# slinderman/pyglm

Measured on AMD Instinct MI355X. Metric: Gibbs sweeps/sec (full resample_model), higher is better.
Workload: dtype f64 (likelihood Gram: exact integer arithmetic on 13 i8 residue planes, CRT back to f64)

## Files before the change

pyglm_amd/csrc/pgl_gemm.hip:

```cpp
#include "pgl_common.h"
#include <type_traits>

namespace {

constexpr int BK = 16;
constexpr int PAD = 16;

template <int WM, int WN, int WZ, bool WEIGHTED, int STAGES = 2>
struct Cfg {
    static constexpr int BM = WM * 64, BN = WN * 64;
    static constexpr int SA = BM + PAD, SB = BN + PAD;
    static constexpr int THREADS = WM * WN * WZ * 64;
    static constexpr int A_ELEMS = BK * SA, B_ELEMS = BK * SB, W_ELEMS = WEIGHTED ? BK * WZ : 0;
    static constexpr int STAGE = A_ELEMS + B_ELEMS + W_ELEMS;
    static constexpr size_t LDS_BYTES = (size_t)STAGES * STAGE * sizeof(double);
    static constexpr int A_LD = (BK * BM / 2) / THREADS, B_LD = (BK * BN / 2) / THREADS;
    static_assert((BK * BM / 2) % THREADS == 0 && (BK * BN / 2) % THREADS == 0, "tile/threads mismatch");
};

__device__ __forceinline__ int isqrt_tri(int t) {
    int r = (int)((__builtin_sqrt(8.0 * (double)t + 1.0) - 1.0) * 0.5);
    while ((long)(r + 1) * (r + 2) / 2 <= t) ++r;
    while ((long)r * (r + 1) / 2 > t) --r;
    return r;
}

__device__ __forceinline__ void block_sync_lds() {
    asm volatile("s_waitcnt lgkmcnt(0)" ::: "memory");
    __builtin_amdgcn_s_barrier();
    asm volatile("" ::: "memory");
}

template <int WM, int WN, int WZ, bool WEIGHTED, int STAGES, bool DMA = false, bool CINIT = false, bool SQ = false>
__device__ __forceinline__ void gemm_item(const PglGemmArgs& g, const long w, double* smem) {
    using C = Cfg<WM, WN, WZ, WEIGHTED, STAGES>;
    const int ntm = (g.M + C::BM - 1) / C::BM;
    int tile, batch, tm, tn;
    if (g.nbatch > 1) {
        if (WEIGHTED || (g.strideA == 0 && g.strideB == 0)) {
            tile = (int)(w / g.nbatch); batch = (int)(w % g.nbatch);
        } else {
            const int ntn_ = (g.N + C::BN - 1) / C::BN;
            const long ntiles = g.tri ? (long)ntm * (ntm + 1) / 2 : (long)ntm * ntn_;
            batch = (int)(w / ntiles); tile = (int)(w % ntiles);
        }
    } else { tile = (int)w; batch = 0; }
    if (g.tri) { tm = isqrt_tri(tile); tn = tile - tm * (tm + 1) / 2; if (g.tri == 2) { const int s_ = tm; tm = tn; tn = s_; } }
    else { tm = tile % ntm; tn = tile / ntm; }
    int Mv = g.M, Nv = g.N;
    if (g.batch_dim) {
        const int d = g.batch_dim[batch] - g.dim_off;
        if (g.dim_mode == 0) { Mv = d; Nv = d; }
        else if (g.dim_mode == 1) Nv = d;
        else if (g.dim_mode == 2) Mv = d;
        else { Mv = g.M < d ? g.M : d; Nv = d; }
    }
    if (tm * C::BM >= Mv || tn * C::BN >= Nv) return;

    int K = g.K;
    if (g.batch_k) { K = g.batch_k[batch]; if (K <= 0) return; }
    const int nkt = K / BK;

    const int tid = threadIdx.x, lane = tid & 63, wave = tid >> 6;
    const int wz = wave / (WM * WN), wmn = wave % (WM * WN), wm = wmn / WN, wn = wmn % WN;
    const int m0 = tm * C::BM, n0 = tn * C::BN;

    const double* __restrict__ Ab = g.A + (long)batch * g.strideA;
    const long roff_ = g.batch_row_off ? (long)g.batch_row_off[batch] : 0;
    const double* __restrict__ Bb = g.B + (long)batch * g.strideB + roff_ * g.ldb;
    const int zg = batch * WZ + wz;
    const bool zvalid = !WEIGHTED || zg < g.nz_total;

    d2_t ra[C::A_LD], rb[C::B_LD];
    double rw = 0.0;
    const unsigned long long aflip = (CINIT && g.alpha < 0.0) ? 0x8000000000000000ull : 0ull;
    typedef unsigned long long u2_t __attribute__((ext_vector_type(2)));
    auto signed_a = [&](d2_t v) { return __builtin_bit_cast(d2_t, __builtin_bit_cast(u2_t, v) ^ u2_t{aflip, aflip}); };
    unsigned oa_[C::A_LD], ob_[C::B_LD], ow_ = 0;
    const char* ka_ = reinterpret_cast<const char*>(Ab);
    const char* kb_ = reinterpret_cast<const char*>(Bb);
    const char* kw_ = reinterpret_cast<const char*>(g.W);
#pragma unroll
    for (int i = 0; i < C::A_LD; ++i) {
        const int p = tid + i * C::THREADS, r = p / (C::BM / 2), c = (p % (C::BM / 2)) * 2;
        int col = m0 + c;
        col = col < g.a_cols ? col : g.a_cols - 2;
        oa_[i] = (unsigned)(((long)r * g.lda + col) * 8);
    }
#pragma unroll
    for (int i = 0; i < C::B_LD; ++i) {
        const int p = tid + i * C::THREADS, r = p / (C::BN / 2), c = (p % (C::BN / 2)) * 2;
        int col = n0 + c;
        col = col < g.b_cols ? col : g.b_cols - 2;
        ob_[i] = (unsigned)(((long)r * g.ldb + col) * 8);
    }
    if (WEIGHTED) {
        const int t_ = tid < BK * WZ ? tid : 0, r = t_ / WZ, z = t_ % WZ;
        int zc = batch * WZ + z;
        zc = zc < g.nz_total ? zc : g.nz_total - 1;
        ow_ = (unsigned)(((long)r * g.ldw + zc) * 8);
    }
    const long stepA = (long)BK * g.lda * 8, stepB = (long)BK * g.ldb * 8, stepW = (long)BK * g.ldw * 8;
    auto gload = [&](int) {
#pragma unroll
        for (int i = 0; i < C::A_LD; ++i) ra[i] = *reinterpret_cast<const d2_t*>(ka_ + oa_[i]);
#pragma unroll
        for (int i = 0; i < C::B_LD; ++i) rb[i] = *reinterpret_cast<const d2_t*>(kb_ + ob_[i]);
        if (WEIGHTED && tid < BK * WZ) rw = *reinterpret_cast<const double*>(kw_ + ow_);
        ka_ += stepA; kb_ += stepB; kw_ += stepW;
    };
    auto lstore = [&](int buf) {
        double* As = smem + buf * C::STAGE;
        double* Bs = As + C::A_ELEMS;
#pragma unroll
        for (int i = 0; i < C::A_LD; ++i) {
            const int p = tid + i * C::THREADS, r = p / (C::BM / 2), c = (p % (C::BM / 2)) * 2;
            if constexpr (CINIT) *reinterpret_cast<d2_t*>(As + r * C::SA + c) = signed_a(SQ ? ra[i] * ra[i] : ra[i]);
            else *reinterpret_cast<d2_t*>(As + r * C::SA + c) = SQ ? ra[i] * ra[i] : ra[i];
        }
#pragma unroll
        for (int i = 0; i < C::B_LD; ++i) {
            const int p = tid + i * C::THREADS, r = p / (C::BN / 2), c = (p % (C::BN / 2)) * 2;
            *reinterpret_cast<d2_t*>(Bs + r * C::SB + c) = SQ ? rb[i] * rb[i] : rb[i];
        }
        if (WEIGHTED && tid < BK * WZ) (Bs + C::B_ELEMS)[tid] = rw;
    };

    d4_t acc[4][4];
    const int frow = lane >> 4, fcol = lane & 15;
    const bool interior = CINIT && m0 + C::BM <= Mv && n0 + C::BN <= Nv;
    if constexpr (CINIT) {
        const double* __restrict__ cp = g.C + (long)batch * g.strideC + roff_ * g.ldc + (long)(m0 + wm * 64 + frow) * g.ldc + (n0 + wn * 64 + fcol);
        if (interior) {
#pragma unroll
            for (int i = 0; i < 4; ++i)
#pragma unroll
                for (int r = 0; r < 4; ++r)
#pragma unroll
                    for (int j = 0; j < 4; ++j) acc[i][j][r] = cp[(long)(i * 16 + 4 * r) * g.ldc + j * 16];
        } else {
#pragma unroll
            for (int i = 0; i < 4; ++i)
#pragma unroll
                for (int r = 0; r < 4; ++r)
#pragma unroll
                    for (int j = 0; j < 4; ++j) {
                        const int row = m0 + wm * 64 + i * 16 + frow + 4 * r, col = n0 + wn * 64 + j * 16 + fcol;
                        acc[i][j][r] = (row < Mv && col < Nv) ? cp[(long)(i * 16 + 4 * r) * g.ldc + j * 16] : 0.0;
                    }
        }
    } else {
#pragma unroll
        for (int i = 0; i < 4; ++i)
#pragma unroll
            for (int j = 0; j < 4; ++j) acc[i][j] = d4_t{0.0, 0.0, 0.0, 0.0};
    }
    auto compute = [&](int buf, int kk) {
        const double* As = smem + buf * C::STAGE + wm * 64 + fcol;
        const double* Bs = smem + buf * C::STAGE + C::A_ELEMS + wn * 64 + fcol;
        const double* Ws = smem + buf * C::STAGE + C::A_ELEMS + C::B_ELEMS;
        const int kr = kk * 4 + frow;
        double a[4], b[4];
#pragma unroll
        for (int i = 0; i < 4; ++i) a[i] = As[kr * C::SA + i * 16];
#pragma unroll
        for (int j = 0; j < 4; ++j) b[j] = Bs[kr * C::SB + j * 16];
        if (WEIGHTED) {
            const double wv = Ws[kr * WZ + wz];
#pragma unroll
            for (int i = 0; i < 4; ++i) a[i] *= wv;
        }
#pragma unroll
        for (int i = 0; i < 4; ++i)
#pragma unroll
            for (int j = 0; j < 4; ++j) acc[i][j] = __builtin_amdgcn_mfma_f64_16x16x4f64(a[i], b[j], acc[i][j], 0, 0, 0);
    };

    if constexpr (STAGES == 2) {
        gload(0);
        lstore(0);
        __syncthreads();
        if constexpr (!WEIGHTED) {
            constexpr int NLD = C::A_LD + C::B_LD;
            static_assert(NLD <= 16, "one staged load per MFMA slot of a k-step");
            auto gload_piece = [&](int q) {
                if (q < C::A_LD) ra[q] = *reinterpret_cast<const d2_t*>(ka_ + oa_[q]);
                else rb[q - C::A_LD] = *reinterpret_cast<const d2_t*>(kb_ + ob_[q - C::A_LD]);
            };
            auto lstore_piece = [&](int buf, int q) {
                double* As = smem + buf * C::STAGE;
                double* Bs = As + C::A_ELEMS;
                if (q < C::A_LD) {
                    const int p = tid + q * C::THREADS, r = p / (C::BM / 2), c = (p % (C::BM / 2)) * 2;
                    if constexpr (CINIT) *reinterpret_cast<d2_t*>(As + r * C::SA + c) = signed_a(SQ ? ra[q] * ra[q] : ra[q]);
                    else *reinterpret_cast<d2_t*>(As + r * C::SA + c) = SQ ? ra[q] * ra[q] : ra[q];
                } else {
                    const int i = q - C::A_LD;
                    const int p = tid + i * C::THREADS, r = p / (C::BN / 2), c = (p % (C::BN / 2)) * 2;
                    *reinterpret_cast<d2_t*>(Bs + r * C::SB + c) = SQ ? rb[i] * rb[i] : rb[i];
                }
            };
            auto kstep = [&](int buf, int kk, auto hook) {
                const double* As = smem + buf * C::STAGE + wm * 64 + fcol;
                const double* Bs = smem + buf * C::STAGE + C::A_ELEMS + wn * 64 + fcol;
                const int kr = kk * 4 + frow;
                double a[4], b[4];
#pragma unroll
                for (int i = 0; i < 4; ++i) a[i] = As[kr * C::SA + i * 16];
#pragma unroll
                for (int j = 0; j < 4; ++j) b[j] = Bs[kr * C::SB + j * 16];
#pragma unroll
                for (int m = 0; m < 16; ++m) {
                    acc[m >> 2][m & 3] = __builtin_amdgcn_mfma_f64_16x16x4f64(a[m >> 2], b[m & 3], acc[m >> 2][m & 3], 0, 0, 0);
                    hook(m);
                    __builtin_amdgcn_sched_barrier(0);
                }
            };
            if constexpr (CINIT && NLD <= 8) {
                double fa0[4], fb0[4], fa1[4], fb1[4];
                auto rd_first = [&](int buf) {
                    const double* As = smem + buf * C::STAGE + wm * 64 + fcol;
                    const double* Bs = smem + buf * C::STAGE + C::A_ELEMS + wn * 64 + fcol;
#pragma unroll
                    for (int i = 0; i < 4; ++i) fa0[i] = As[frow * C::SA + i * 16];
#pragma unroll
                    for (int j = 0; j < 4; ++j) fb0[j] = Bs[frow * C::SB + j * 16];
                };
                auto kstep_a = [&](int buf, auto kk_c, auto hook) {
                    constexpr int KK = decltype(kk_c)::value;
                    double (&ca)[4] = (KK & 1) ? fa1 : fa0;
                    double (&cb)[4] = (KK & 1) ? fb1 : fb0;
                    double (&na)[4] = (KK & 1) ? fa0 : fa1;
                    double (&nb)[4] = (KK & 1) ? fb0 : fb1;
                    const double* As = smem + buf * C::STAGE + wm * 64 + fcol;
                    const double* Bs = smem + buf * C::STAGE + C::A_ELEMS + wn * 64 + fcol;
                    const int krn = (KK + 1) * 4 + frow;
#pragma unroll
                    for (int m = 0; m < 16; ++m) {
                        asm volatile("v_mfma_f64_16x16x4_f64 %0, %1, %2, %0" : "+a"(acc[m >> 2][m & 3]) : "v"(ca[m >> 2]), "v"(cb[m & 3]));
                        if constexpr (KK < 3) {
                            if (m < 4) na[m] = As[krn * C::SA + m * 16];
                            else if (m < 8) nb[m - 4] = Bs[krn * C::SB + (m - 4) * 16];
                        }
                        hook(m);
                        __builtin_amdgcn_sched_barrier(0);
                    }
                };
                using K0 = std::integral_constant<int, 0>; using K1 = std::integral_constant<int, 1>;
                using K2 = std::integral_constant<int, 2>; using K3 = std::integral_constant<int, 3>;
                auto nohook = [](int) {};
                rd_first(0);
                asm volatile("s_nop 7\n\ts_nop 7" ::: "memory");
                for (int kt = 0; kt + 1 < nkt; ++kt) {
                    const int buf = kt & 1;
                    kstep_a(buf, K0{}, [&](int m) { if (m >= 8 && m - 8 < NLD) gload_piece(m - 8); });
                    ka_ += stepA; kb_ += stepB;
                    kstep_a(buf, K1{}, nohook);
                    kstep_a(buf, K2{}, nohook);
                    kstep_a(buf, K3{}, [&](int m) { if (m >= 16 - NLD) lstore_piece(buf ^ 1, m - (16 - NLD)); });
                    __syncthreads();
                    rd_first(buf ^ 1);
                }
                {
                    const int buf = (nkt - 1) & 1;
                    kstep_a(buf, K0{}, nohook);
                    kstep_a(buf, K1{}, nohook);
                    kstep_a(buf, K2{}, nohook);
                    kstep_a(buf, K3{}, nohook);
                }
                asm volatile("s_nop 7\n\ts_nop 7\n\ts_nop 7" ::: "memory");
            } else {
            for (int kt = 0; kt + 1 < nkt; ++kt) {
                const int buf = kt & 1;
                kstep(buf, 0, [&](int m) { if (m < NLD) gload_piece(m); });
                ka_ += stepA; kb_ += stepB;
                compute(buf, 1);
                compute(buf, 2);
                kstep(buf, 3, [&](int m) { if (m >= 16 - NLD) lstore_piece(buf ^ 1, m - (16 - NLD)); });
                __syncthreads();
            }
            {
                const int buf = (nkt - 1) & 1;
#pragma unroll
                for (int kk = 0; kk < BK / 4; ++kk) compute(buf, kk);
            }
            }
        } else {
            for (int kt = 0; kt < nkt; ++kt) {
                const int buf = kt & 1;
                if (kt + 1 < nkt) gload(kt + 1);
#pragma unroll
                for (int kk = 0; kk < BK / 4; ++kk) compute(buf, kk);
                if (kt + 1 < nkt) lstore(buf ^ 1);
                __syncthreads();
            }
        }
    } else {
        static_assert(DMA && WEIGHTED && (STAGES == 3 || STAGES == 4), "the 3/4-stage pipeline is the DMA-staged weighted Gram");
        typedef __attribute__((address_space(3))) void* lds_ptr_t;
        typedef const __attribute__((address_space(1))) void* glb_ptr_t;
        static_assert(C::BM == 128 && C::BN == 128 && C::THREADS == 512, "DMA staging is written for the Gram tile");
        const int wv = __builtin_amdgcn_readfirstlane(wave);
        const char* gp[5];
        long gstep[5];
        int loff[5];
        {
            int ca = m0 + lane * 2, cb = n0 + lane * 2;
            ca = ca < g.a_cols ? ca : g.a_cols - 2;
            cb = cb < g.b_cols ? cb : g.b_cols - 2;
#pragma unroll
            for (int p = 0; p < 4; ++p) {
                const int r = wv + 8 * (p >> 1);
                if ((p & 1) == 0) { gp[p] = reinterpret_cast<const char*>(Ab + (long)r * g.lda + ca); gstep[p] = (long)BK * g.lda * 8; loff[p] = r * C::SA * 8; }
                else { gp[p] = reinterpret_cast<const char*>(Bb + (long)r * g.ldb + cb); gstep[p] = (long)BK * g.ldb * 8; loff[p] = (C::A_ELEMS + r * C::SB) * 8; }
            }
            const int dw = wv * 8 + (lane & 7), dbl = dw >> 1, r = dbl / WZ, zq = dbl % WZ;
            int zc = batch * WZ + zq;
            zc = zc < g.nz_total ? zc : g.nz_total - 1;
            gp[4] = reinterpret_cast<const char*>(g.W + (long)r * g.ldw + zc) + 4 * (dw & 1);
            gstep[4] = (long)BK * g.ldw * 8;
            loff[4] = (C::A_ELEMS + C::B_ELEMS) * 8 + wv * 32;
        }
        long gadv[5];
        auto advance = [&](bool adv) {
#pragma unroll
            for (int p = 0; p < 5; ++p) gadv[p] = adv ? gstep[p] : 0;
        };
        auto dma_piece = [&](int stage, int p) {
            char* dst = reinterpret_cast<char*>(smem) + (size_t)stage * C::STAGE * 8 + loff[p];
            if (p < 4) __builtin_amdgcn_global_load_lds((glb_ptr_t)gp[p], (lds_ptr_t)dst, 16, 0, 0);
            else if (lane < 8) __builtin_amdgcn_global_load_lds((glb_ptr_t)gp[4], (lds_ptr_t)dst, 4, 0, 0);
            asm volatile("v_lshl_add_u64 %0, %1, 0, %2" : "=v"(gp[p]) : "v"(gp[p]), "s"(gadv[p]));
        };
        auto dma = [&](int stage) {
#pragma unroll
            for (int p = 0; p < 5; ++p) dma_piece(stage, p);
        };
        advance(1 < nkt);
        dma(0);
        advance(2 < nkt);
        dma(1);
        if constexpr (STAGES == 4) { advance(3 < nkt); dma(2); }
        advance(STAGES < nkt);
        if constexpr (STAGES == 4) asm volatile("s_waitcnt vmcnt(10)" ::: "memory");
        else asm volatile("s_waitcnt vmcnt(5)" ::: "memory");
        __syncthreads();
        int cur = 0;
        {
            const int wq = wmn;
            double pa[2][2][2], pb[2][2][8], pw[2][2];
            auto rdA = [&](int buf, int kk, int i) { return smem[buf * C::STAGE + wq * 32 + fcol + (kk * 4 + frow) * C::SA + i * 16]; };
            auto rdB = [&](int buf, int kk, int j) { return smem[buf * C::STAGE + C::A_ELEMS + fcol + (kk * 4 + frow) * C::SB + j * 16]; };
            auto rdW = [&](int buf, int kk) { return smem[buf * C::STAGE + C::A_ELEMS + C::B_ELEMS + (kk * 4 + frow) * WZ + wz]; };
#pragma unroll
            for (int i = 0; i < 2; ++i) { pa[0][0][i] = rdA(0, 0, i); pa[0][1][i] = rdA(0, 1, i); }
#pragma unroll
            for (int j = 0; j < 8; ++j) pb[0][0][j] = rdB(0, 0, j);
            pw[0][0] = rdW(0, 0); pw[0][1] = rdW(0, 1);
#pragma unroll
            for (int i = 0; i < 2; ++i) { pa[0][0][i] *= pw[0][0]; pa[0][1][i] *= pw[0][1]; }
            for (int kt = 0; kt < nkt; ++kt) {
                const int nxt = (cur == STAGES - 1) ? 0 : cur + 1;
                const int dstage = (cur == 0) ? STAGES - 1 : cur - 1;
                if (kt + STAGES >= nkt) advance(false);
#pragma unroll
                for (int p = 0; p < 2; ++p) {
                    const int ps = p, ns = p ^ 1;
                    const int nbuf = (p == 0) ? cur : nxt, nk = (p == 0) ? 2 : 0;
#pragma unroll
                    for (int m = 0; m < 16; ++m) {
                        const int i = m >> 3, j = m & 7;
                        acc[m >> 2][m & 3] = __builtin_amdgcn_mfma_f64_16x16x4f64(pa[ps][0][i], pb[ps][0][j], acc[m >> 2][m & 3], 0, 0, 0);
                        if (m < 8) pb[ps][1][m] = rdB(cur, 2 * p + 1, m);
                        else if (m < 10) pa[ns][0][m - 8] = rdA(nbuf, nk, m - 8);
                        else if (m == 10) pw[ns][0] = rdW(nbuf, nk);
                        else if (m == 11) pw[ns][1] = rdW(nbuf, nk + 1);
                        else { if (p == 1) dma_piece(dstage, m - 12); }
                        __builtin_amdgcn_sched_barrier(0);
                    }
#pragma unroll
                    for (int m = 0; m < 16; ++m) {
                        const int i = m >> 3, j = m & 7;
                        acc[m >> 2][m & 3] = __builtin_amdgcn_mfma_f64_16x16x4f64(pa[ps][1][i], pb[ps][1][j], acc[m >> 2][m & 3], 0, 0, 0);
                        if (m < 2) pa[ns][1][m] = rdA(nbuf, nk + 1, m);
                        else if (m < 10) pb[ns][0][m - 2] = rdB(nbuf, nk, m - 2);
                        else if (m == 10) { if (p == 1) dma_piece(dstage, 4); }
                        else if (m == 13) {
#pragma unroll
                            for (int q = 0; q < 2; ++q) { pa[ns][0][q] *= pw[ns][0]; pa[ns][1][q] *= pw[ns][1]; }
                        }
                        __builtin_amdgcn_sched_barrier(0);
                    }
                    if (p == 0) {
                        if constexpr (STAGES == 4) asm volatile("s_waitcnt vmcnt(5)" ::: "memory");
                        else asm volatile("s_waitcnt vmcnt(0)" ::: "memory");
                        block_sync_lds();
                    }
                }
                cur = nxt;
            }
        }
    }

    if (!zvalid) return;
    double* __restrict__ Cb = g.C + (WEIGHTED ? (long)zg : (long)batch) * g.strideC + roff_ * g.ldc;
    const double alpha = g.alpha, beta = g.beta;
    constexpr bool WIDE = STAGES >= 3;
    auto roff = [&](int i, int j) { return WIDE ? wmn * 32 + ((4 * i + j) >> 3) * 16 : wm * 64 + i * 16; };
    auto coff = [&](int i, int j) { return WIDE ? ((4 * i + j) & 7) * 16 : wn * 64 + j * 16; };
    if constexpr (CINIT) {
        double* __restrict__ cq = Cb + (long)(m0 + wm * 64 + frow) * g.ldc + (n0 + wn * 64 + fcol);
        if (interior) {
#pragma unroll
            for (int i = 0; i < 4; ++i)
#pragma unroll
                for (int r = 0; r < 4; ++r)
#pragma unroll
                    for (int j = 0; j < 4; ++j) cq[(long)(i * 16 + 4 * r) * g.ldc + j * 16] = acc[i][j][r];
        } else {
#pragma unroll
            for (int i = 0; i < 4; ++i)
#pragma unroll
                for (int r = 0; r < 4; ++r)
#pragma unroll
                    for (int j = 0; j < 4; ++j) {
                        const int row = m0 + wm * 64 + i * 16 + frow + 4 * r, col = n0 + wn * 64 + j * 16 + fcol;
                        if (row < Mv && col < Nv) cq[(long)(i * 16 + 4 * r) * g.ldc + j * 16] = acc[i][j][r];
                    }
        }
        return;
    }
#pragma unroll
    for (int i = 0; i < 4; ++i) {
        double cv[4][4];
        if (beta != 0.0) {
#pragma unroll
            for (int r = 0; r < 4; ++r) {
#pragma unroll
                for (int j = 0; j < 4; ++j) {
                    const int row = m0 + roff(i, j) + frow + 4 * r, col = n0 + coff(i, j) + fcol;
                    cv[r][j] = (row < Mv && col < Nv) ? Cb[(long)row * g.ldc + col] : 0.0;
                }
            }
        }
#pragma unroll
        for (int r = 0; r < 4; ++r) {
#pragma unroll
            for (int j = 0; j < 4; ++j) {
                const int row = m0 + roff(i, j) + frow + 4 * r, col = n0 + coff(i, j) + fcol;
                if (row >= Mv || col >= Nv) continue;
                double v = alpha * acc[i][j][r];
                if (beta != 0.0) v += beta * cv[r][j];
                Cb[(long)row * g.ldc + col] = v;
            }
        }
    }
}

template <int WM, int WN, int WZ, bool WEIGHTED, int STAGES, bool CINIT = false, bool SQ = false>
__global__ __launch_bounds__(WM* WN* WZ * 64, 2) void gemm_tn_f64(PglGemmArgs g) {
    using C = Cfg<WM, WN, WZ, WEIGHTED, STAGES>;
    extern __shared__ __attribute__((aligned(16))) double smem[];
    const int ntm = (g.M + C::BM - 1) / C::BM, ntn = (g.N + C::BN - 1) / C::BN;
    const long total = (long)(g.tri ? ntm * (ntm + 1) / 2 : ntm * ntn) * g.nbatch;
    const long chunk = (total + 7) / 8;
    long w = (long)(blockIdx.x & 7) * chunk + (blockIdx.x >> 3);
    if ((long)(blockIdx.x >> 3) >= chunk || w >= total) return;
    gemm_item<WM, WN, WZ, WEIGHTED, STAGES, false, CINIT, SQ>(g, w, smem);
}

template <int WM, int WN, int WZ, bool WEIGHTED, int STAGES, bool DMA>
__global__ __launch_bounds__(WM* WN* WZ * 64, 2) void gemm_tn_f64_persistent(PglGemmArgs g) {
    using C = Cfg<WM, WN, WZ, WEIGHTED, STAGES>;
    extern __shared__ __attribute__((aligned(16))) double smem[];
    long* ticket = reinterpret_cast<long*>(smem + (size_t)STAGES * C::STAGE);
    const int ntm = (g.M + C::BM - 1) / C::BM, ntn = (g.N + C::BN - 1) / C::BN;
    const long total = (long)(g.tri ? ntm * (ntm + 1) / 2 : ntm * ntn) * g.nbatch;
    const long chunk = (total + 7) / 8;
    unsigned xcc;
    asm volatile("s_getreg_b32 %0, hwreg(HW_REG_XCC_ID)" : "=s"(xcc));
    xcc &= 7u;
    for (;;) {
        __syncthreads();
        if (threadIdx.x == 0) {
            long w = -1;
            for (int hop = 0; hop < 8 && w < 0; ++hop) {
                const int y = (int)((xcc + hop) & 7u);
                const long lo = (long)y * chunk, hi = (lo + chunk < total) ? lo + chunk : total;
                if (lo >= hi) continue;
                const long it = atomicAdd(&g.sched[y], 1);
                if (lo + it < hi) w = lo + it;
            }
            ticket[0] = w;
        }
        __syncthreads();
        const long w = ticket[0];
        if (w < 0) break;
        gemm_item<WM, WN, WZ, WEIGHTED, STAGES, DMA>(g, w, smem);
    }
}

constexpr int FK = 8, FST = 4, FSA = 128 + PAD;
constexpr int F_A = FK * FSA, F_B = FK * FSA, F_W = FK;
constexpr int F_STAGE = F_A + F_B + F_W;
constexpr size_t F_LDS = (size_t)FST * F_STAGE * sizeof(double) + 16;

__device__ __forceinline__ void gram_fine_item(const PglGemmArgs& g, const long w, double* smem) {
    typedef __attribute__((address_space(3))) void* lds_ptr_t;
    typedef const __attribute__((address_space(1))) void* glb_ptr_t;
    const int nz = g.nz_total;
    const int z = (int)(w % nz);
    const int S = g.ksplit > 1 ? g.ksplit : 1;
    const int sl = (int)((w / nz) % S), tile = (int)(w / nz / S);
    const int tm = isqrt_tri(tile), tn = tile - tm * (tm + 1) / 2;
    const int m0 = tm * 128, n0 = tn * 128;
    const long krow0 = S > 1 ? (long)sl * g.ks_rows : 0;
    const int Ks = S > 1 ? (int)((long)g.K - krow0 < g.ks_rows ? (long)g.K - krow0 : g.ks_rows) : g.K;
    const int nkt = Ks / FK;
    const int tid = threadIdx.x, lane = tid & 63, wq = tid >> 6;
    const int frow = lane >> 4, fcol = lane & 15;
    const double* __restrict__ Ab = g.A + krow0 * g.lda;
    const double* __restrict__ Bb = g.B + krow0 * g.ldb;

    const int wv = __builtin_amdgcn_readfirstlane(wq);
    const char* gp[5];
    long gstep[5], gadv[5];
    int loff[5];
    {
        int ca = m0 + lane * 2, cb = n0 + lane * 2;
        ca = ca < g.a_cols ? ca : g.a_cols - 2;
        cb = cb < g.b_cols ? cb : g.b_cols - 2;
#pragma unroll
        for (int p = 0; p < 4; ++p) {
            const int r = wv + 4 * (p >> 1);
            if ((p & 1) == 0) { gp[p] = reinterpret_cast<const char*>(Ab + (long)r * g.lda + ca); gstep[p] = (long)FK * g.lda * 8; loff[p] = r * FSA * 8; }
            else { gp[p] = reinterpret_cast<const char*>(Bb + (long)r * g.ldb + cb); gstep[p] = (long)FK * g.ldb * 8; loff[p] = (F_A + r * FSA) * 8; }
        }
        const int dw = wv * 4 + (lane & 3), r = dw >> 1;
        gp[4] = reinterpret_cast<const char*>(g.W + (krow0 + r) * g.ldw + z) + 4 * (dw & 1);
        gstep[4] = (long)FK * g.ldw * 8;
        loff[4] = (F_A + F_B) * 8 + wv * 16;
    }
    auto advance = [&](bool adv) {
#pragma unroll
        for (int p = 0; p < 5; ++p) gadv[p] = adv ? gstep[p] : 0;
    };
    auto dma_piece = [&](int stage, int p) {
        char* dst = reinterpret_cast<char*>(smem) + (size_t)stage * F_STAGE * 8 + loff[p];
        if (p < 4) __builtin_amdgcn_global_load_lds((glb_ptr_t)gp[p], (lds_ptr_t)dst, 16, 0, 0);
        else if (lane < 4) __builtin_amdgcn_global_load_lds((glb_ptr_t)gp[4], (lds_ptr_t)dst, 4, 0, 0);
        gp[p] += gadv[p];
    };
    auto dma = [&](int stage) {
#pragma unroll
        for (int p = 0; p < 5; ++p) dma_piece(stage, p);
    };

    d4_t acc[4][4];
#pragma unroll
    for (int i = 0; i < 4; ++i)
#pragma unroll
        for (int j = 0; j < 4; ++j) acc[i][j] = d4_t{0.0, 0.0, 0.0, 0.0};

    advance(1 < nkt); dma(0);
    advance(2 < nkt); dma(1);
    advance(3 < nkt); dma(2);
    asm volatile("s_waitcnt vmcnt(5)" ::: "memory");
    block_sync_lds();

    double pa[2][2][2], pb[2][2][8], pw[2][2];
    auto rdA = [&](int buf, int kk, int i) { return smem[buf * F_STAGE + wq * 32 + fcol + (kk * 4 + frow) * FSA + i * 16]; };
    auto rdB = [&](int buf, int kk, int j) { return smem[buf * F_STAGE + F_A + fcol + (kk * 4 + frow) * FSA + j * 16]; };
    auto rdW = [&](int buf, int kk) { return smem[buf * F_STAGE + F_A + F_B + kk * 4 + frow]; };
#pragma unroll
    for (int i = 0; i < 2; ++i) { pa[0][0][i] = rdA(0, 0, i); pa[0][1][i] = rdA(0, 1, i); }
#pragma unroll
    for (int j = 0; j < 8; ++j) pb[0][0][j] = rdB(0, 0, j);
    pw[0][0] = rdW(0, 0); pw[0][1] = rdW(0, 1);
#pragma unroll
    for (int i = 0; i < 2; ++i) { pa[0][0][i] *= pw[0][0]; pa[0][1][i] *= pw[0][1]; }

    int cur = 0;
    for (int kt0 = 0; kt0 < nkt; kt0 += 2) {
#pragma unroll
        for (int p = 0; p < 2; ++p) {
            const int kt = kt0 + p;
            if (kt >= nkt) break;
            const int ps = p, ns = p ^ 1;
            const int nxt = (cur + 1) & (FST - 1), dstage = (cur + 3) & (FST - 1);
            advance(kt + 4 < nkt);
#pragma unroll
            for (int m = 0; m < 16; ++m) {
                const int i = m >> 3, j = m & 7;
                acc[m >> 2][m & 3] = __builtin_amdgcn_mfma_f64_16x16x4f64(pa[ps][0][i], pb[ps][0][j], acc[m >> 2][m & 3], 0, 0, 0);
                if (m < 8) pb[ps][1][m] = rdB(cur, 1, m);
                else if (m < 10) pa[ns][0][m - 8] = rdA(nxt, 0, m - 8);
                else if (m == 10) pw[ns][0] = rdW(nxt, 0);
                else if (m == 11) pw[ns][1] = rdW(nxt, 1);
                else dma_piece(dstage, m - 12);
                __builtin_amdgcn_sched_barrier(0);
            }
#pragma unroll
            for (int m = 0; m < 16; ++m) {
                const int i = m >> 3, j = m & 7;
                acc[m >> 2][m & 3] = __builtin_amdgcn_mfma_f64_16x16x4f64(pa[ps][1][i], pb[ps][1][j], acc[m >> 2][m & 3], 0, 0, 0);
                if (m < 2) pa[ns][1][m] = rdA(nxt, 1, m);
                else if (m < 10) pb[ns][0][m - 2] = rdB(nxt, 0, m - 2);
                else if (m == 10) dma_piece(dstage, 4);
                else if (m == 13) {
#pragma unroll
                    for (int q = 0; q < 2; ++q) { pa[ns][0][q] *= pw[ns][0]; pa[ns][1][q] *= pw[ns][1]; }
                }
                __builtin_amdgcn_sched_barrier(0);
            }
            asm volatile("s_waitcnt vmcnt(5)" ::: "memory");
            block_sync_lds();
            cur = nxt;
        }
    }

    double* __restrict__ Cb = S > 1 ? g.Cpart + (long)z * g.part_stride_z + (long)sl * g.part_stride_s : g.C + (long)z * g.strideC;
    const double alpha = S > 1 ? 1.0 : g.alpha, beta = S > 1 ? 0.0 : g.beta;
#pragma unroll
    for (int i = 0; i < 4; ++i) {
        double cv[4][4];
        if (beta != 0.0) {
#pragma unroll
            for (int r = 0; r < 4; ++r)
#pragma unroll
                for (int j = 0; j < 4; ++j) {
                    const int f = 4 * i + j;
                    const int row = m0 + wq * 32 + (f >> 3) * 16 + frow + 4 * r, col = n0 + (f & 7) * 16 + fcol;
                    cv[r][j] = (row < g.M && col < g.N) ? Cb[(long)row * g.ldc + col] : 0.0;
                }
        }
#pragma unroll
        for (int r = 0; r < 4; ++r)
#pragma unroll
            for (int j = 0; j < 4; ++j) {
                const int f = 4 * i + j;
                const int row = m0 + wq * 32 + (f >> 3) * 16 + frow + 4 * r, col = n0 + (f & 7) * 16 + fcol;
                if (row >= g.M || col >= g.N) continue;
                double v = alpha * acc[i][j][r];
                if (beta != 0.0) v += beta * cv[r][j];
                Cb[(long)row * g.ldc + col] = v;
            }
    }
}

__global__ __launch_bounds__(256, 2) void gram_fine_persistent(PglGemmArgs g) {
    extern __shared__ __attribute__((aligned(16))) double smem[];
    long* ticket = reinterpret_cast<long*>(smem + (size_t)FST * F_STAGE);
    const int ntm = (g.M + 127) / 128;
    const long total = (long)ntm * (ntm + 1) / 2 * g.nz_total * (g.ksplit > 1 ? g.ksplit : 1);
    const long chunk = (total + 7) / 8;
    unsigned xcc;
    asm volatile("s_getreg_b32 %0, hwreg(HW_REG_XCC_ID)" : "=s"(xcc));
    xcc &= 7u;
    for (;;) {
        __syncthreads();
        if (threadIdx.x == 0) {
            long w = -1;
            for (int hop = 0; hop < 8 && w < 0; ++hop) {
                const int y = (int)((xcc + hop) & 7u);
                const long lo = (long)y * chunk, hi = (lo + chunk < total) ? lo + chunk : total;
                if (lo >= hi) continue;
                const long it = atomicAdd(&g.sched[y], 1);
                if (lo + it < hi) w = lo + it;
            }
            ticket[0] = w;
        }
        __syncthreads();
        const long w = ticket[0];
        if (w < 0) break;
        gram_fine_item(g, w, smem);
    }
}

template <int WM, int WN, int WZ, bool WEIGHTED, int STAGES = 2, bool CINIT = false, bool SQ = false>
int launch(const PglGemmArgs& a, hipStream_t st) {
    using C = Cfg<WM, WN, WZ, WEIGHTED, STAGES>;
    if constexpr (!WEIGHTED && STAGES == 2 && !CINIT) {
        if (a.beta == 1.0 && (a.alpha == 1.0 || a.alpha == -1.0)) return launch<WM, WN, WZ, WEIGHTED, STAGES, true, SQ>(a, st);
    }
    static PglPerDevice attr_set;
    auto kern = gemm_tn_f64<WM, WN, WZ, WEIGHTED, STAGES, CINIT, SQ>;
    if (int rc = pgl_set_dynamic_lds(reinterpret_cast<const void*>(kern), C::LDS_BYTES, attr_set)) return rc;
    const int ntm = (a.M + C::BM - 1) / C::BM, ntn = (a.N + C::BN - 1) / C::BN;
    const long ntiles = a.tri ? (long)ntm * (ntm + 1) / 2 : (long)ntm * ntn;
    const long total = ntiles * a.nbatch;
    if (total <= 0) return PGL_OK;
    const long chunk = (total + 7) / 8;
    const long grid = chunk * 8;
    if (grid > 0x7fffffffL) { pgl_set_error("gemm grid too large: %ld", grid); return PGL_ERR_ARG; }
    hipLaunchKernelGGL(kern, dim3((unsigned)grid), dim3(C::THREADS), C::LDS_BYTES, st, a);
    PGL_CHECK_LAUNCH();
    return PGL_OK;
}

static int* sched_slot(hipStream_t st) {
    static std::atomic<int*> bases[PGL_MAX_DEVICES];
    static std::atomic<unsigned> next{0};
    constexpr unsigned SLOTS = 256;
    std::atomic<int*>& b = bases[pgl_device() & (PGL_MAX_DEVICES - 1)];
    int* base = b.load(std::memory_order_acquire);
    if (!base) {
        int* fresh = nullptr;
        if (hipMalloc(reinterpret_cast<void**>(&fresh), SLOTS * 8 * sizeof(int)) != hipSuccess) return nullptr;
        if (b.compare_exchange_strong(base, fresh, std::memory_order_acq_rel)) base = fresh;
        else (void)hipFree(fresh);
    }
    int* slot = base + (size_t)(next.fetch_add(1, std::memory_order_relaxed) % SLOTS) * 8;
    if (hipMemsetAsync(slot, 0, 8 * sizeof(int), st) != hipSuccess) return nullptr;
    return slot;
}

template <int WM, int WN, int WZ, bool WEIGHTED, int STAGES, bool DMA>
int launch_persistent(const PglGemmArgs& a0, hipStream_t st) {
    using C = Cfg<WM, WN, WZ, WEIGHTED, STAGES>;
    static PglPerDevice attr_set;
    auto kern = gemm_tn_f64_persistent<WM, WN, WZ, WEIGHTED, STAGES, DMA>;
    constexpr size_t lds = C::LDS_BYTES + 16;
    if (int rc = pgl_set_dynamic_lds(reinterpret_cast<const void*>(kern), lds, attr_set)) return rc;
    const int n_cu = pgl_device_cus(pgl_device());
    const int ntm = (a0.M + C::BM - 1) / C::BM, ntn = (a0.N + C::BN - 1) / C::BN;
    const long total = (a0.tri ? (long)ntm * (ntm + 1) / 2 : (long)ntm * ntn) * a0.nbatch;
    if (total <= 0) return PGL_OK;
    PglGemmArgs a = a0;
    a.sched = sched_slot(st);
    if (!a.sched) { pgl_set_error("persistent gemm: scheduler scratch unavailable"); return PGL_ERR_HIP; }
    const long per_cu = (lds * 2 <= 160 * 1024) ? 2 : 1;
    const long grid = total < n_cu * per_cu ? total : n_cu * per_cu;
    hipLaunchKernelGGL(kern, dim3((unsigned)grid), dim3(C::THREADS), lds, st, a);
    PGL_CHECK_LAUNCH();
    return PGL_OK;
}

static int launch_gram_fine(const PglGemmArgs& a0, hipStream_t st) {
    static PglPerDevice attr_set;
    if (int rc = pgl_set_dynamic_lds(reinterpret_cast<const void*>(gram_fine_persistent), F_LDS, attr_set)) return rc;
    const int n_cu = pgl_device_cus(pgl_device());
    const int ntm = (a0.M + 127) / 128;
    const long total = (long)ntm * (ntm + 1) / 2 * a0.nz_total * (a0.ksplit > 1 ? a0.ksplit : 1);
    if (total <= 0) return PGL_OK;
    PglGemmArgs a = a0;
    a.sched = sched_slot(st);
    if (!a.sched) { pgl_set_error("persistent gemm: scheduler scratch unavailable"); return PGL_ERR_HIP; }
    const long grid = total < 2L * n_cu ? total : 2L * n_cu;
    hipLaunchKernelGGL(gram_fine_persistent, dim3((unsigned)grid), dim3(256), F_LDS, st, a);
    PGL_CHECK_LAUNCH();
    return PGL_OK;
}

}

int* pgl_sched_slot(hipStream_t st) { return sched_slot(st); }

namespace {
__global__ __launch_bounds__(256) void sum_k_slices_kernel(const double* __restrict__ part, long stride_z, long stride_s, int S, double* __restrict__ C,
                                                           long strideC, long ldc, int M, int accumulate) {
    const long e = (long)blockIdx.x * 256 + threadIdx.x;
    if (e >= (long)M * M) return;
    const int r = (int)(e / M), c = (int)(e % M), z = blockIdx.y;
    if (r / 128 < c / 128) return;
    const double* p = part + (long)z * stride_z + (long)r * ldc + c;
    double* out = C + (long)z * strideC + (long)r * ldc + c;
    double acc = accumulate ? *out : 0.0;
    for (int s = 0; s < S; ++s) acc += p[(long)s * stride_s];
    *out = acc;
}
}

int pgl_gram_split(const double* X, long ldx, int x_cols, const double* W, long ldw, int Tp, int D, int nz, double* J, long ldj, long strideJ, int accumulate,
                   long ks_rows, double* part, long part_stride_z, hipStream_t st) {
    PGL_CHECK_ARG(X && W && J && part && Tp > 0 && Tp % 16 == 0 && D > 0 && D <= 512 && nz > 0 && ldj >= D && ldw >= nz && ks_rows >= 16 && ks_rows % 16 == 0);
    const int S = (int)((Tp + ks_rows - 1) / ks_rows);
    PGL_CHECK_ARG(S >= 2 && part_stride_z >= (long)S * ldj * ldj);
    PglGemmArgs a{};
    a.A = X; a.lda = ldx; a.B = X; a.ldb = ldx;
    a.C = J; a.ldc = ldj; a.strideC = strideJ;
    a.W = W; a.ldw = ldw;
    a.M = D; a.N = D; a.K = Tp;
    a.a_cols = x_cols & ~1; a.b_cols = x_cols & ~1;
    a.nbatch = (nz + 1) / 2; a.nz_total = nz;
    a.alpha = 1.0; a.beta = 0.0; a.tri = 1;
    a.ksplit = S; a.ks_rows = ks_rows; a.Cpart = part; a.part_stride_z = part_stride_z; a.part_stride_s = ldj * ldj;
    PGL_CHECK_ARG(((uintptr_t)a.A % 16) == 0 && a.lda % 2 == 0);
    if (int rc = launch_gram_fine(a, st)) return rc;
    hipLaunchKernelGGL(sum_k_slices_kernel, dim3((unsigned)(((long)D * D + 255) / 256), nz), dim3(256), 0, st, part, part_stride_z, a.part_stride_s, S, J, strideJ, ldj, D,
                       accumulate);
    PGL_CHECK_LAUNCH();
    return PGL_OK;
}


int pgl_launch_gemm(PglGemmKind kind, const PglGemmArgs& a, hipStream_t st) {
    PGL_CHECK_ARG(a.K % BK == 0 && a.M > 0 && a.N > 0 && a.nbatch > 0);
    PGL_CHECK_ARG(a.a_cols % 2 == 0 && a.b_cols % 2 == 0 && a.lda % 2 == 0 && a.ldb % 2 == 0);
    PGL_CHECK_ARG(((uintptr_t)a.A % 16) == 0 && ((uintptr_t)a.B % 16) == 0);
    if (a.pipe && kind != PGL_GEMM_GRAM2) {
        if ((a.pipe == 2 || a.beta == 0.0) && pgl_update_supported(a)) return pgl_launch_update(a, st);
    }
    switch (kind) {
        case PGL_GEMM_GRAM2: PGL_CHECK_ARG(a.W != nullptr && a.tri == 1 && a.M == a.N && a.batch_dim == nullptr); {
            const int n_cu = pgl_device_cus(pgl_device());
            const long ntm = (a.M + 127) / 128;
            if (ntm * (ntm + 1) / 2 * a.nbatch < 2L * n_cu) return launch_gram_fine(a, st);
            return launch_persistent<2, 2, 2, true, 3, true>(a, st);
        }
        case PGL_GEMM_PLAIN:
            PGL_CHECK_ARG(a.tri == 0);
            if (a.N <= 128) return launch<2, 2, 1, false>(a, st);
            if (a.M <= 64) return launch<1, 4, 1, false>(a, st);
            return launch<2, 4, 1, false>(a, st);
        case PGL_GEMM_SQUARES:
            PGL_CHECK_ARG(a.tri == 0 && !a.pipe);
            if (a.M <= 64) return launch<1, 4, 1, false, 2, false, true>(a, st);
            return launch<2, 4, 1, false, 2, false, true>(a, st);
        case PGL_GEMM_TRI1: {
            PGL_CHECK_ARG(a.M == a.N);
            const int extra = a.M % 128;
            if (a.pipe && a.tri == 1 && a.batch_dim == nullptr && a.M > 128 && extra >= 1 && extra <= 16 && pgl_update_supported(a)) {
                if (int rc = pgl_launch_update_rows(a, a.M - extra, extra, st)) return rc;
                PglGemmArgs b = a;
                b.M = b.N = a.M - extra;
                return launch<2, 2, 1, false>(b, st);
            }
            return launch<2, 2, 1, false>(a, st);
        }
    }
    pgl_set_error("unknown gemm kind %d", (int)kind);
    return PGL_ERR_ARG;
}
```

Baseline: 0.05775.

## Skip dead MFMA sub-tiles on diagonal and edge tiles, rebalancing waves

For the CINIT read-modify-write GEMM path with 2x2 waves, diagonal tiles of triangular (syrk-like) products now remap wave offsets so the upper/lower triangle's live 16x16 sub-blocks are spread evenly across the four waves. A per-wave live mask also covers out-of-bounds edge sub-blocks, and each MFMA is guarded by a scalar branch on that mask. Dead sub-tiles are neither loaded nor stored from C. This removes wasted matrix-core work on diagonal and ragged tiles. It adds a scalar compare and branch per MFMA, which could cost issue slots on full interior tiles.

```diff
diff --git a/pyglm_amd/csrc/pgl_gemm.hip b/pyglm_amd/csrc/pgl_gemm.hip
--- a/pyglm_amd/csrc/pgl_gemm.hip
+++ b/pyglm_amd/csrc/pgl_gemm.hip
@@ -30,6 +30,8 @@
     __builtin_amdgcn_s_barrier();
     asm volatile("" ::: "memory");
 }
+
+#define PGL_MFMA_F64_IF "s_cmp_eq_u32 %3, 0\n\ts_cbranch_scc1 .Lpgl_skip%=\n\tv_mfma_f64_16x16x4_f64 %0, %1, %2, %0\n.Lpgl_skip%=:"
 
 template <int WM, int WN, int WZ, bool WEIGHTED, int STAGES, bool DMA = false, bool CINIT = false, bool SQ = false>
 __device__ __forceinline__ void gemm_item(const PglGemmArgs& g, const long w, double* smem) {
@@ -128,9 +130,30 @@
 
     d4_t acc[4][4];
     const int frow = lane >> 4, fcol = lane & 15;
-    const bool interior = CINIT && m0 + C::BM <= Mv && n0 + C::BN <= Nv;
+    constexpr bool RMW_AGPR = CINIT && !WEIGHTED && STAGES == 2 && C::A_LD + C::B_LD <= 8;
+    constexpr bool BALANCED = RMW_AGPR && WM == 2 && WN == 2 && WZ == 1;
+    const bool diag = BALANCED && g.tri != 0 && tm == tn;
+    const bool upper = g.tri == 2;
+    const bool interior = CINIT && !diag && m0 + C::BM <= Mv && n0 + C::BN <= Nv;
+    int ro = wm * 64, co = wn * 64;
+    unsigned e_live = 0xffffu;
+    if constexpr (RMW_AGPR) {
+        const int sw = __builtin_amdgcn_readfirstlane(wmn), swm = sw / WN, swn = sw % WN;
+        ro = swm * 64; co = swn * 64;
+        if (diag) {
+            if (swm == swn) e_live = upper ? 0x8cefu : 0xf731u;
+            else if (!upper) { ro = 64; co = 0; e_live = swm ? 0x00ffu : 0xff00u; }
+            else { ro = 0; co = 64; e_live = swn ? 0x3333u : 0xccccu; }
+        }
+        const int nrb = min(4, max(0, (Mv - m0 - ro + 15) >> 4)), ncb = min(4, max(0, (Nv - n0 - co + 15) >> 4));
+        e_live = __builtin_amdgcn_readfirstlane(e_live & (((1u << ncb) - 1u) * (0x1111u & ((1u << 4 * nrb) - 1u))));
+    }
+    auto c_live = [&](int i, int j, int row, int col) {
+        if constexpr (RMW_AGPR) return row < Mv && col < Nv && ((e_live >> (4 * i + j)) & 1u) && (!diag || (upper ? col >= row : col <= row));
+        else return row < Mv && col < Nv;
+    };
     if constexpr (CINIT) {
-        const double* __restrict__ cp = g.C + (long)batch * g.strideC + roff_ * g.ldc + (long)(m0 + wm * 64 + frow) * g.ldc + (n0 + wn * 64 + fcol);
+        const double* __restrict__ cp = g.C + (long)batch * g.strideC + roff_ * g.ldc + (long)(m0 + ro + frow) * g.ldc + (n0 + co + fcol);
         if (interior) {
 #pragma unroll
             for (int i = 0; i < 4; ++i)
@@ -145,8 +168,8 @@
                 for (int r = 0; r < 4; ++r)
 #pragma unroll
                     for (int j = 0; j < 4; ++j) {
-                        const int row = m0 + wm * 64 + i * 16 + frow + 4 * r, col = n0 + wn * 64 + j * 16 + fcol;
-                        acc[i][j][r] = (row < Mv && col < Nv) ? cp[(long)(i * 16 + 4 * r) * g.ldc + j * 16] : 0.0;
+                        const int row = m0 + ro + i * 16 + frow + 4 * r, col = n0 + co + j * 16 + fcol;
+                        acc[i][j][r] = c_live(i, j, row, col) ? cp[(long)(i * 16 + 4 * r) * g.ldc + j * 16] : 0.0;
                     }
         }
     } else {
@@ -219,8 +242,8 @@
             if constexpr (CINIT && NLD <= 8) {
                 double fa0[4], fb0[4], fa1[4], fb1[4];
                 auto rd_first = [&](int buf) {
-                    const double* As = smem + buf * C::STAGE + wm * 64 + fcol;
-                    const double* Bs = smem + buf * C::STAGE + C::A_ELEMS + wn * 64 + fcol;
+                    const double* As = smem + buf * C::STAGE + ro + fcol;
+                    const double* Bs = smem + buf * C::STAGE + C::A_ELEMS + co + fcol;
 #pragma unroll
                     for (int i = 0; i < 4; ++i) fa0[i] = As[frow * C::SA + i * 16];
 #pragma unroll
@@ -232,12 +255,12 @@
                     double (&cb)[4] = (KK & 1) ? fb1 : fb0;
                     double (&na)[4] = (KK & 1) ? fa0 : fa1;
                     double (&nb)[4] = (KK & 1) ? fb0 : fb1;
-                    const double* As = smem + buf * C::STAGE + wm * 64 + fcol;
-                    const double* Bs = smem + buf * C::STAGE + C::A_ELEMS + wn * 64 + fcol;
+                    const double* As = smem + buf * C::STAGE + ro + fcol;
+                    const double* Bs = smem + buf * C::STAGE + C::A_ELEMS + co + fcol;
                     const int krn = (KK + 1) * 4 + frow;
 #pragma unroll
                     for (int m = 0; m < 16; ++m) {
-                        asm volatile("v_mfma_f64_16x16x4_f64 %0, %1, %2, %0" : "+a"(acc[m >> 2][m & 3]) : "v"(ca[m >> 2]), "v"(cb[m & 3]));
+                        asm volatile(PGL_MFMA_F64_IF : "+a"(acc[m >> 2][m & 3]) : "v"(ca[m >> 2]), "v"(cb[m & 3]), "s"(e_live & (1u << m)) : "scc");
                         if constexpr (KK < 3) {
                             if (m < 4) na[m] = As[krn * C::SA + m * 16];
                             else if (m < 8) nb[m - 4] = Bs[krn * C::SB + (m - 4) * 16];
@@ -409,7 +432,7 @@
     auto roff = [&](int i, int j) { return WIDE ? wmn * 32 + ((4 * i + j) >> 3) * 16 : wm * 64 + i * 16; };
     auto coff = [&](int i, int j) { return WIDE ? ((4 * i + j) & 7) * 16 : wn * 64 + j * 16; };
     if constexpr (CINIT) {
-        double* __restrict__ cq = Cb + (long)(m0 + wm * 64 + frow) * g.ldc + (n0 + wn * 64 + fcol);
+        double* __restrict__ cq = Cb + (long)(m0 + ro + frow) * g.ldc + (n0 + co + fcol);
         if (interior) {
 #pragma unroll
             for (int i = 0; i < 4; ++i)
@@ -424,8 +447,8 @@
                 for (int r = 0; r < 4; ++r)
 #pragma unroll
                     for (int j = 0; j < 4; ++j) {
-                        const int row = m0 + wm * 64 + i * 16 + frow + 4 * r, col = n0 + wn * 64 + j * 16 + fcol;
-                        if (row < Mv && col < Nv) cq[(long)(i * 16 + 4 * r) * g.ldc + j * 16] = acc[i][j][r];
+                        const int row = m0 + ro + i * 16 + frow + 4 * r, col = n0 + co + j * 16 + fcol;
+                        if (c_live(i, j, row, col)) cq[(long)(i * 16 + 4 * r) * g.ldc + j * 16] = acc[i][j][r];
                     }
         }
         return;
```

After: 0.05781 (median of 3 runs). About the same (+0.1%).
